# microsoft/tutel

Measured on NVIDIA H100. Metric: moe_layer_fwd_bwd_tokens_per_sec, higher is better.
Workload: dtype bf16; 1 GPU; model=helloworld moe_layer top-2 8-expert ffn(relu) model_dim=4096 hidden=14336, global_batch=16, seq_len=512, parallelism=ep1 (8 local experts/GPU), a2a_ffn_overlap_degree=1, cuda_graph=True, launches_per_graph_replay=15

## Files before the change

### csrc/gemm_sm90.cu

```cuda
#include "gemm_sm90.h"

#include <cuda.h>
#include <cuda_bf16.h>
#include <cuda_fp16.h>

#include <cstdio>
#include <cstdlib>
#include <mutex>

#include "ptx.cuh"

namespace tb {

struct GemmArgs {
  int M, N, K, G;
  int b_group_div;
  int tiles_m, tiles_n;
  long long num_tiles;

  void* d;
  long long ldd, d_group_stride;
  const unsigned long long* d_ptr_table;
  int out_dtype;

// ... 78 lines not shown
  const int first_m = band * kBand;
  const int rows_in_band = min(kBand, tiles_m - first_m);
  r -= band * band_tiles;
  c.m_blk = first_m + r % rows_in_band;
  c.n_blk = r / rows_in_band;
  return c;
}

__device__ __forceinline__ int rotate_group(int g, int rot, int mod) {
  if (mod > 1) {
    const int base = (g / mod) * mod;
    return base + (g - base + rot) % mod;
  }
  if (mod < -1) {
    const int m = -mod;
    const int base = (g / m) * m;
    return base + (rot + m - (g - base)) % m;
  }
  return g;
}

__device__ __forceinline__ float gelu_erf(float x) { return 0.5f * x * (1.0f + erff(x * 0.70710678118654752f)); }
__device__ __forceinline__ float silu(float x) { return __fdividef(x, 1.0f + __expf(-x)); }
__device__ __forceinline__ float fast_sigmoid(float x) { return __fdividef(1.0f, 1.0f + __expf(-x)); }
__device__ __forceinline__ float relu_bwd(float v, float x) { return x > 0.0f ? v : 0.0f; }
__device__ __forceinline__ float gelu_bwd(float v, float x) {
  const float cdf = 0.5f * (1.0f + erff(x * 0.70710678118654752f));
  return v * (cdf + x * 0.3989422804014327f * __expf(-0.5f * x * x));
}
__device__ __forceinline__ float silu_bwd(float v, float x) {
  const float sg = fast_sigmoid(x);
  return v * (sg * (1.0f + x * (1.0f - sg)));
}
__device__ __forceinline__ uint32_t pack2(float a, float b, bool bf16) {
  const __nv_bfloat162 hb = __floats2bfloat162_rn(a, b);
  const __half2 hh = __floats2half2_rn(a, b);
  return bf16 ? *reinterpret_cast<const uint32_t*>(&hb) : *reinterpret_cast<const uint32_t*>(&hh);
}
__device__ __forceinline__ float2 unpack2(uint32_t w, bool bf16) {
  const float2 h = __half22float2(*reinterpret_cast<const __half2*>(&w));
  return bf16 ? make_float2(__uint_as_float(w << 16), __uint_as_float(w & 0xFFFF0000u)) : h;
}

__device__ __forceinline__ void unpack8(const uint4& u, bool is_bf16, float* f) {
  const uint32_t w[4] = {u.x, u.y, u.z, u.w};
#pragma unroll
  for (int i = 0; i < 4; ++i) {
    if (is_bf16) {
      f[2 * i] = __uint_as_float(w[i] << 16);
      f[2 * i + 1] = __uint_as_float(w[i] & 0xFFFF0000u);
    } else {
      const __half2 h = *reinterpret_cast<const __half2*>(&w[i]);
      const float2 t = __half22float2(h);
      f[2 * i] = t.x;
      f[2 * i + 1] = t.y;
    }
  }
}
template <bool BF16>
__device__ __forceinline__ void pack32_t(const float* v, uint32_t* w) {
#pragma unroll
  for (int i = 0; i < 16; ++i) {
    if constexpr (BF16) {
      const __nv_bfloat162 h = __floats2bfloat162_rn(v[2 * i], v[2 * i + 1]);
      w[i] = *reinterpret_cast<const uint32_t*>(&h);
    } else {
      const __half2 h = __floats2half2_rn(v[2 * i], v[2 * i + 1]);
      w[i] = *reinterpret_cast<const uint32_t*>(&h);
    }
  }
}
__device__ __forceinline__ void pack32(const float* v, uint32_t* w, bool is_bf16) {
  if (is_bf16) pack32_t<true>(v, w); else pack32_t<false>(v, w);
}
// ... 29 lines not shown
    else a = g[j] * fast_sigmoid(g[j]);
    o[j] = a * u[j];
  }
}
template <int ACT>
__device__ __forceinline__ void glu_bwd_seg(const float* r, const float* g, float* u, float* o) {
#pragma unroll
  for (int j = 0; j < 32; ++j) {
    const float dh = r[j];
    float a, da;
    if constexpr (ACT == ACT_RELU) {
      a = fmaxf(g[j], 0.0f);
      da = g[j] > 0.0f ? 1.0f : 0.0f;
    } else if constexpr (ACT == ACT_GELU) {
      const float cdf = 0.5f * (1.0f + erff(g[j] * 0.70710678118654752f));
      a = g[j] * cdf;
      da = cdf + g[j] * 0.3989422804014327f * __expf(-0.5f * g[j] * g[j]);
    } else {
      const float sg = fast_sigmoid(g[j]);
      a = g[j] * sg;
      da = sg * (1.0f + g[j] * (1.0f - sg));
    }
    o[j] = dh * u[j] * da;
    u[j] = dh * a;
  }
}

enum WideMain : int { WM_NONE, WM_BIAS, WM_RELU_BWD, WM_ADD, WM_GELU_BWD, WM_SILU_BWD };

__device__ __forceinline__ uint32_t out_tile_off(int j, int swz) {
  return static_cast<uint32_t>((j >> 3) * (128 * kSwizzleBytes) + (((j & 7) ^ swz) << 4));
}

__device__ __forceinline__ void wide_scale(float (&acc)[128], float sa0, float sa1, const float* sb, int n_lane, int n_lim) {
#pragma unroll
  for (int j = 0; j < 32; ++j) {
    const int n = n_lane + 8 * j;
    if (sb != nullptr && n < n_lim) {
      const float2 s = *reinterpret_cast<const float2*>(sb + n);
      acc[4 * j] *= sa0 * s.x; acc[4 * j + 1] *= sa0 * s.y;
      acc[4 * j + 2] *= sa1 * s.x; acc[4 * j + 3] *= sa1 * s.y;
    } else {
      acc[4 * j] *= sa0; acc[4 * j + 1] *= sa0;
      acc[4 * j + 2] *= sa1; acc[4 * j + 3] *= sa1;
    }
  }
}

template <int WM>
__device__ __forceinline__ void wide_main(float (&acc)[128], const uint8_t* row0, int swz, const uint8_t* bias_s,
                                          bool bias_f32, bool bias_bf16, int n_lane, int n_lim, bool out_bf16, float alpha) {
#pragma unroll
  for (int j = 0; j < 32; ++j) {
    if constexpr (WM == WM_NONE) {
#pragma unroll
      for (int c = 0; c < 4; ++c) acc[4 * j + c] *= alpha;
    } else if constexpr (WM == WM_BIAS) {
      const int n = n_lane + 8 * j;
      float2 b = make_float2(0.0f, 0.0f);
      if (n < n_lim)
        b = bias_f32 ? *reinterpret_cast<const float2*>(bias_s + n * 4)
                     : unpack2(*reinterpret_cast<const uint32_t*>(bias_s + n * 2), bias_bf16);
      acc[4 * j] += b.x; acc[4 * j + 1] += b.y;
      acc[4 * j + 2] += b.x; acc[4 * j + 3] += b.y;
    } else {
      const uint32_t o = out_tile_off(j, swz);
#pragma unroll
      for (int h = 0; h < 2; ++h) {
        const float2 f = unpack2(*reinterpret_cast<const uint32_t*>(row0 + h * 8 * kSwizzleBytes + o), out_bf16);
        float& v0 = acc[4 * j + 2 * h];
        float& v1 = acc[4 * j + 2 * h + 1];
        if constexpr (WM == WM_RELU_BWD) { v0 = relu_bwd(v0, f.x); v1 = relu_bwd(v1, f.y); }
        else if constexpr (WM == WM_ADD) { v0 += f.x; v1 += f.y; }
        else if constexpr (WM == WM_GELU_BWD) { v0 = gelu_bwd(v0, f.x); v1 = gelu_bwd(v1, f.y); }
        else { v0 = silu_bwd(v0, f.x); v1 = silu_bwd(v1, f.y); }
      }
    }
  }
}

template <int ACT>
__device__ __forceinline__ void wide_act(float (&acc)[128]) {
#pragma unroll
  for (int i = 0; i < 128; ++i) {
    if constexpr (ACT == ACT_RELU) acc[i] = fmaxf(acc[i], 0.0f);
    else if constexpr (ACT == ACT_GELU) acc[i] = gelu_erf(acc[i]);
    else acc[i] = silu(acc[i]);
  }
}

__device__ __forceinline__ void wide_stage(const float (&acc)[128], uint8_t* row0, int swz, bool out_bf16) {
#pragma unroll
  for (int j = 0; j < 32; ++j) {
    const uint32_t o = out_tile_off(j, swz);
    *reinterpret_cast<uint32_t*>(row0 + o) = pack2(acc[4 * j], acc[4 * j + 1], out_bf16);
    *reinterpret_cast<uint32_t*>(row0 + 8 * kSwizzleBytes + o) = pack2(acc[4 * j + 2], acc[4 * j + 3], out_bf16);
  }
}

template <int OFF>
__device__ __forceinline__ void colsum_halve(float (&s)[64], int lane) {
  const bool upper = (lane & OFF) != 0;
#pragma unroll
  for (int i = 0; i < 2 * OFF; ++i) {
    const float lo = s[i], hi = s[i + 2 * OFF];
    const float recv = __shfl_xor_sync(0xffffffffu, upper ? lo : hi, OFF);
    s[i] = (upper ? hi : lo) + recv;
  }
}
__device__ __forceinline__ void wide_colsum(const float (&acc)[128], bool ok0, bool ok1, int lane, float* colrow) {
  float s[64];
#pragma unroll
  for (int j = 0; j < 32; ++j) {
#pragma unroll
    for (int c = 0; c < 2; ++c) s[2 * j + c] = (ok0 ? acc[4 * j + c] : 0.0f) + (ok1 ? acc[4 * j + 2 + c] : 0.0f);
  }
  colsum_halve<16>(s, lane);
  colsum_halve<8>(s, lane);
  colsum_halve<4>(s, lane);
  float* base = colrow + 32 * (lane >> 2) + 2 * (lane & 3);
#pragma unroll
  for (int q = 0; q < 4; ++q) *reinterpret_cast<float2*>(base + 8 * q) = make_float2(s[2 * q], s[2 * q + 1]);
}

__device__ __forceinline__ void hand_over_tile(const uint8_t* tile, bool straddle, int m0, int n0, int m_valid, int N, int g,
                                               long long group_stride, long long ld, uint8_t* dst, int ct, int lane,
                                               uint32_t out_full) {
  constexpr int kChunks = 256 / 8;
  ptx::fence_proxy_async_smem();
  if (straddle) {
    ptx::named_bar_sync(1, 256);
    for (int i = ct; i < 128 * kChunks; i += 256) {
      const int r = i / kChunks, ch = i % kChunks;
      const int m = m0 + r, n = n0 + ch * 8;
      if (m < m_valid && n < N) {
        const uint4 v = *reinterpret_cast<const uint4*>(tile + (ch >> 3) * (128 * kSwizzleBytes) + r * kSwizzleBytes +
                                                        (((ch & 7) ^ (r & 7)) << 4));
        *reinterpret_cast<uint4*>(dst + (static_cast<long long>(g) * group_stride + static_cast<long long>(m) * ld + n) * 2) = v;
      }
    }
  }
  __syncwarp();
  if (lane == 0) ptx::mbar_arrive(out_full);
}

template <int BN_, bool A_MN, bool B_MN, int DT>
__global__ void __maxnreg__(Cfg<BN_>::MAXNREG)
gemm_sm90_kernel(const __grid_constant__ CUtensorMap tmA, const __grid_constant__ CUtensorMap tmB,
                 const __grid_constant__ CUtensorMap tmB2, const __grid_constant__ CUtensorMap tmD,
                 const __grid_constant__ CUtensorMap tmAux, const __grid_constant__ CUtensorMap tmD2,
                 const GemmArgs args) {
  using C = Cfg<BN_>;
  constexpr int BN = C::BN;
  extern __shared__ uint8_t smem_raw[];

  const int warp = __shfl_sync(0xffffffffu, static_cast<int>(threadIdx.x >> 5), 0);
  const int lane = threadIdx.x & 31;

  const uint32_t smem_base = (ptx::smem_u32(smem_raw) + 1023u) & ~1023u;
  constexpr int stages = C::STAGES;
  const uint32_t out_base = smem_base + static_cast<uint32_t>(stages) * C::STAGE_BYTES;
  const uint32_t bar_base = out_base + C::OUT_TILE_BYTES;
  auto smem_a = [&](int s) { return smem_base + s * C::STAGE_BYTES; };
  auto smem_b = [&](int s) { return smem_base + s * C::STAGE_BYTES + C::A_BYTES; };
  auto full_bar = [&](int s) { return bar_base + 8u * s; };
  auto empty_bar = [&](int s) { return bar_base + 64u + 8u * s; };
  const uint32_t aux_full = bar_base + 128u;
  const uint32_t out_empty = bar_base + 136u;
  const uint32_t out_full = bar_base + 144u;
  auto side_full = [&](uint32_t slot) { return bar_base + 152u + 8u * slot; };
  const uint32_t epi_base = bar_base + C::BAR_BYTES;
  float* epi_ptr = reinterpret_cast<float*>(smem_raw + (epi_base - ptx::smem_u32(smem_raw)));
  uint8_t* out_tile = smem_raw + (out_base - ptx::smem_u32(smem_raw));
  float* colsum_part = epi_ptr;
  const uint32_t side_base = epi_base + C::COLSUM_BYTES;
  const bool aux_tma = C::WIDE && (args.epilogue == EPI_RELU_BWD || args.epilogue == EPI_ADD || args.epilogue == EPI_ACT_BWD);
  const bool side_bias = C::WIDE && args.bias != nullptr && !aux_tma && args.epilogue != EPI_NONE;
  const bool side_in = side_bias || (C::WIDE && args.scale_b != nullptr);
  const bool pre_act = C::WIDE && args.d2 != nullptr && (args.epilogue == EPI_BIAS_GELU || args.epilogue == EPI_BIAS_SILU);
// ... 71 lines not shown
            constexpr int chunk_elems = kSwizzleBytes / kEltBytes;
            constexpr int chunk_bytes = bk_elems * kSwizzleBytes;
            if constexpr (!A_MN) {
              ptx::tma_load_3d(smem_a(s), &tmA, fb, k0, m0, tc.g);
            } else {
              for (int c = 0; c < C::BM / chunk_elems; ++c)
                ptx::tma_load_3d(smem_a(s) + c * chunk_bytes, &tmA, fb, m0 + c * chunk_elems, k0, tc.g);
            }
            if (!dual) {
              if constexpr (!B_MN) {
                ptx::tma_load_3d(smem_b(s), &tmB, fb, k0, n0, gb);
              } else {
                for (int c = 0; c < BN / chunk_elems; ++c)
                  ptx::tma_load_3d(smem_b(s) + c * chunk_bytes, &tmB, fb, n0 + c * chunk_elems, k0, gb);
              }
            } else {
              const int nb0 = tc.n_blk * (BN / 2);
              if constexpr (!B_MN) {
                ptx::tma_load_3d(smem_b(s), &tmB, fb, k0, nb0, gb);
                ptx::tma_load_3d(smem_b(s) + (BN / 2) * kSwizzleBytes, &tmB2, fb, k0, nb0, gb);
              } else {
                constexpr int half_chunks = (BN / 2) / chunk_elems;
                for (int c = 0; c < 2 * half_chunks; ++c)
                  ptx::tma_load_3d(smem_b(s) + c * chunk_bytes, c < half_chunks ? &tmB : &tmB2, fb,
                                   nb0 + (c % half_chunks) * chunk_elems, k0, gb);
              }
            }
          }
          __syncwarp();
          if (++s == stages) { s = 0; ph ^= 1u; }
        }
      }
    } else if (C::WIDE && warp == 1) {
      const int side_es = args.bias_is_fp32 ? 4 : 2;
      uint32_t it = 0;
      uint32_t outs = 0;
      TileCoord prev{};
      int prev_m_valid = 0;
      auto drain = [&](const CUtensorMap* map, const TileCoord& tc, int m_valid, bool colsum, bool has_next, TileCoord next) {
        const int m0 = tc.m_blk * C::BM, n0 = tc.n_blk * BN;
        const bool straddle = m0 + C::BM > m_valid && m_valid < args.M;
        ptx::mbar_wait_quiet(out_full, outs & 1u);
        if (!straddle && lane == 0) {
          for (int b = 0; b < BN / 64; ++b)
            if (n0 + 64 * b < args.N) ptx::tma_store_3d(map, out_base + b * C::OUT_BOX_BYTES, n0 + 64 * b, m0, tc.g);
          ptx::bulk_commit_group();
        }
        if (colsum) {
#pragma unroll 1
          for (int h = 0; h < 2; ++h) {
            const int c = 128 * h + 4 * lane;
            float4 v = *reinterpret_cast<const float4*>(colsum_part + c);
#pragma unroll
            for (int w = 1; w < 8; ++w) {
              const float4 p = *reinterpret_cast<const float4*>(colsum_part + w * BN + c);
              v.x += p.x; v.y += p.y; v.z += p.z; v.w += p.w;
            }
            const int n = n0 + c;
            if (n < args.N) {
              float* cs = args.colsum + static_cast<long long>(tc.g / args.b_group_div) * args.colsum_group_stride + n;
              if ((reinterpret_cast<uintptr_t>(cs) & 15) == 0) {
                ptx::red_add_v4_f32(cs, v.x, v.y, v.z, v.w);
              } else {
                atomicAdd(cs, v.x); atomicAdd(cs + 1, v.y); atomicAdd(cs + 2, v.z); atomicAdd(cs + 3, v.w);
              }
            }
          }
// ... 60 lines not shown
    ptx::setmaxnreg_inc<C::CONSUMER_REGS>();
    const int cw = warp - 4;
    const int wg = cw >> 2;
    const bool wg_leader = (threadIdx.x & 127) == 0;
    int s = 0;
    uint32_t ph = 0;
    constexpr uint32_t kMnChunkBytes = 64u * kSwizzleBytes;
    constexpr uint32_t kMnKStep = 16u * kSwizzleBytes;
    constexpr uint32_t a_lbo = A_MN ? kMnChunkBytes : 16u;
    constexpr uint32_t b_lbo = B_MN ? kMnChunkBytes : 16u;
    constexpr uint32_t a_kstep = (A_MN ? kMnKStep : 32u) >> 4;
    constexpr uint32_t b_kstep = (B_MN ? kMnKStep : 32u) >> 4;
    constexpr uint32_t desc_hi = (1024u >> 4) | (1u << 30);
    const uint32_t a_lo0 = (((smem_a(0) + static_cast<uint32_t>(wg) * 8192u) >> 4) & 0x3FFFu) | ((a_lbo >> 4) << 16);
    const uint32_t b_lo0 = ((smem_b(0) >> 4) & 0x3FFFu) | ((b_lbo >> 4) << 16);

    const bool out16 = (args.out_dtype != DT_FP32);
    const bool out_bf16 = (args.out_dtype == DT_BF16);
    const bool glu = !C::WIDE && (args.epilogue == EPI_GLU || args.epilogue == EPI_GLU_BWD);
    float* epi_warp = epi_ptr + cw * 16 * C::EPI_PITCH;
    const float* epi_row = epi_warp + (lane & 15) * C::EPI_PITCH;
    const int col_half = (lane >> 4) * 32;
    auto load_acc = [&](int col, float* v) {
#pragma unroll
      for (int q = 0; q < 8; ++q) {
        const float4 t4 = *reinterpret_cast<const float4*>(epi_row + col + q * 4);
        v[q * 4] = t4.x; v[q * 4 + 1] = t4.y; v[q * 4 + 2] = t4.z; v[q * 4 + 3] = t4.w;
      }
    };
    const int ct = threadIdx.x - 128;
    const int r0 = cw * 16 + (lane >> 2);
    const int swz = lane >> 2;
    uint8_t* row0 = out_tile + r0 * kSwizzleBytes + (lane & 3) * 4;
    const int wmain = args.epilogue == EPI_NONE ? WM_NONE
                    : args.epilogue == EPI_ADD ? WM_ADD
                    : args.epilogue == EPI_RELU_BWD ? WM_RELU_BWD
                    : args.epilogue == EPI_ACT_BWD ? (args.act == ACT_GELU ? WM_GELU_BWD : args.act == ACT_SILU ? WM_SILU_BWD : WM_RELU_BWD)
                    : WM_BIAS;
    uint32_t it = 0;
    uint32_t outs = 0;

    for (long long t = tile_first; t < args.num_tiles; t += tile_step) {
      TileCoord tc = decode_tile<kBand>(t, args.tiles_m, args.tiles_n);
      tc.g = rotate_group(tc.g, args.group_rot, args.group_mod);
      int m_valid = args.M;
      if (args.row_counts != nullptr) {
        m_valid = min(args.M, args.row_counts[tc.g]);
        if (tc.m_blk * C::BM >= m_valid) continue;
      }
      float acc[BN / 2];
      if constexpr (C::WIDE) {
#pragma unroll
        for (int i = 0; i < BN / 2; ++i) acc[i] = 0.0f;
      }
      int prev_s = 0;
      for (int kb = 0; kb < num_kb; ++kb) {
        ptx::mbar_wait_quiet(full_bar(s), ph);
        const uint32_t a_lo = a_lo0 + static_cast<uint32_t>(s) * (C::STAGE_BYTES >> 4);
        const uint32_t b_lo = b_lo0 + static_cast<uint32_t>(s) * (C::STAGE_BYTES >> 4);
        ptx::wgmma_fence();
#pragma unroll
        for (int k = 0; k < 4; ++k) {
          const uint64_t ad = (static_cast<uint64_t>(desc_hi) << 32) | (a_lo + k * a_kstep);
          const uint64_t bd = (static_cast<uint64_t>(desc_hi) << 32) | (b_lo + k * b_kstep);
          if constexpr (BN == 256) ptx::wgmma_m64n256<DT, A_MN, B_MN>(acc, ad, bd, (kb | k) != 0);
          else ptx::wgmma_m64n128<DT, A_MN, B_MN>(acc, ad, bd, (kb | k) != 0);
        }
        ptx::wgmma_commit();
        if (kb > 0) {
          ptx::wgmma_wait<1>();
          if (wg_leader) ptx::mbar_arrive(empty_bar(prev_s));
        }
        prev_s = s;
        if (++s == stages) { s = 0; ph ^= 1u; }
      }
      ptx::wgmma_wait<0>();
      if (wg_leader) ptx::mbar_arrive(empty_bar(prev_s));

      if constexpr (C::WIDE) {
        const int m0 = tc.m_blk * C::BM, n0 = tc.n_blk * BN;
        const bool ok0 = m0 + r0 < m_valid, ok1 = m0 + r0 + 8 < m_valid;
        const int n_lane = 2 * (lane & 3);
        const int n_lim = args.N - n0;
        const bool straddle = m0 + C::BM > m_valid && m_valid < args.M;
        const uint8_t* side = reinterpret_cast<const uint8_t*>(colsum_part + 8 * BN) + (it & 1u) * C::SIDE_SLOT_BYTES;
        if (side_in) ptx::mbar_wait_quiet(side_full(it & 1u), (it >> 1) & 1u);
        if (args.scale_a != nullptr || args.scale_b != nullptr) {
          const float* sa = args.scale_a != nullptr ? args.scale_a + static_cast<long long>(tc.g) * args.scale_a_group_stride + m0 + r0 : nullptr;
          const float sa0 = (sa != nullptr && ok0) ? sa[0] : 1.0f;
          const float sa1 = (sa != nullptr && ok1) ? sa[8] : 1.0f;
          const float* sb = args.scale_b != nullptr ? reinterpret_cast<const float*>(side + C::SIDE_BIAS_BYTES) : nullptr;
          wide_scale(acc, sa0, sa1, sb, n_lane, n_lim);
        }
        auto wait_out_free = [&]() { ptx::mbar_wait_quiet(out_empty, (outs & 1u) ^ 1u); };
        auto hand_over = [&](uint8_t* dst) {
          hand_over_tile(out_tile, straddle, m0, n0, m_valid, args.N, tc.g, args.d_group_stride, args.ldd, dst, ct, lane, out_full);
          ++outs;
        };

        if (wmain == WM_BIAS) {
          if (side_bias)
            wide_main<WM_BIAS>(acc, row0, swz, side, args.bias_is_fp32 != 0, args.bias_is_bf16 != 0, n_lane, n_lim, out_bf16, 1.0f);
          if (pre_act) {
            wait_out_free();
            wide_stage(acc, row0, swz, out_bf16);
            hand_over(reinterpret_cast<uint8_t*>(args.d2));
          }
          if (args.epilogue == EPI_BIAS_RELU) wide_act<ACT_RELU>(acc);
          else if (args.epilogue == EPI_BIAS_GELU) wide_act<ACT_GELU>(acc);
          else if (args.epilogue == EPI_BIAS_SILU) wide_act<ACT_SILU>(acc);
        } else if (wmain == WM_NONE) {
          if (args.alpha != 1.0f) wide_main<WM_NONE>(acc, row0, swz, nullptr, false, false, n_lane, n_lim, out_bf16, args.alpha);
        } else {
          ptx::mbar_wait_quiet(aux_full, it & 1u);
          if (wmain == WM_RELU_BWD) wide_main<WM_RELU_BWD>(acc, row0, swz, nullptr, false, false, n_lane, n_lim, out_bf16, 1.0f);
          else if (wmain == WM_ADD) wide_main<WM_ADD>(acc, row0, swz, nullptr, false, false, n_lane, n_lim, out_bf16, 1.0f);
          else if (wmain == WM_GELU_BWD) wide_main<WM_GELU_BWD>(acc, row0, swz, nullptr, false, false, n_lane, n_lim, out_bf16, 1.0f);
          else wide_main<WM_SILU_BWD>(acc, row0, swz, nullptr, false, false, n_lane, n_lim, out_bf16, 1.0f);
        }
        if (!aux_tma) wait_out_free();
        wide_stage(acc, row0, swz, out_bf16);
        if (args.colsum != nullptr) wide_colsum(acc, ok0, ok1, lane, colsum_part + cw * BN);
        hand_over(reinterpret_cast<uint8_t*>(args.d));
        ++it;
        continue;
      }

      {
        const int fr = lane >> 2, fc = (lane & 3) * 2;
#pragma unroll
        for (int j = 0; j < C::EPI_COLS / 8; ++j) {
          *reinterpret_cast<float2*>(epi_warp + fr * C::EPI_PITCH + j * 8 + fc) = make_float2(acc[4 * j], acc[4 * j + 1]);
          *reinterpret_cast<float2*>(epi_warp + (fr + 8) * C::EPI_PITCH + j * 8 + fc) = make_float2(acc[4 * j + 2], acc[4 * j + 3]);
        }
      }
      __syncwarp();

      const int m = tc.m_blk * C::BM + cw * 16 + (lane & 15);
      const bool row_ok = m < m_valid;
      const int gb = tc.g / args.b_group_div;
      uint8_t* d_base = (args.d_ptr_table != nullptr)
                            ? reinterpret_cast<uint8_t*>(args.d_ptr_table[tc.g])
                            : reinterpret_cast<uint8_t*>(args.d) +
                                  static_cast<long long>(tc.g) * args.d_group_stride * (out16 ? 2 : 4);
      uint8_t* d_row = d_base + static_cast<long long>(m) * args.ldd * (out16 ? 2 : 4);
      const uint8_t* aux_row = nullptr;
      if (args.aux != nullptr)
        aux_row = reinterpret_cast<const uint8_t*>(args.aux) +
                  (static_cast<long long>(tc.g) * args.aux_group_stride + static_cast<long long>(m) * args.ld_aux) * 2;
      const uint8_t* aux2_row = nullptr;
      if (args.aux2 != nullptr)
        aux2_row = reinterpret_cast<const uint8_t*>(args.aux2) +
                   (static_cast<long long>(tc.g) * args.aux_group_stride + static_cast<long long>(m) * args.ld_aux) * 2;
      const uint8_t* bias_g = nullptr;
      if (args.bias != nullptr)
// ... 234 lines not shown
  }
  dims[2] = static_cast<cuuint64_t>(groups);
  box[2] = 1;
  strides[0] = static_cast<cuuint64_t>(ld) * eb;
  strides[1] = static_cast<cuuint64_t>(groups > 1 ? group_stride : (mn_major ? k : rows_mn) * ld) * eb;
  if (strides[1] == 0) strides[1] = strides[0];
  CUresult r = enc(map, dt, 3, const_cast<void*>(base), dims, strides, box, estr, CU_TENSOR_MAP_INTERLEAVE_NONE,
                   CU_TENSOR_MAP_SWIZZLE_128B, CU_TENSOR_MAP_L2_PROMOTION_L2_256B, CU_TENSOR_MAP_FLOAT_OOB_FILL_NONE);
  if (r != CUDA_SUCCESS) { *why = "cuTensorMapEncodeTiled failed"; return false; }
  return true;
}

bool make_tile_map(CUtensorMap* map, const void* base, int dtype, long long rows, long long cols, long long ld,
                   long long group_stride, int groups, const char** why) {
  EncodeTiledFn enc = get_encode_fn();
  if (enc == nullptr) { *why = "cuTensorMapEncodeTiled unavailable"; return false; }
  if ((reinterpret_cast<uintptr_t>(base) & 15) || ((ld * 2) & 15) || ((group_stride * 2) & 15)) {
    *why = "output / aux base and strides must be 16-byte aligned";
    return false;
  }
  const cuuint64_t dims[3] = {static_cast<cuuint64_t>(cols), static_cast<cuuint64_t>(rows), static_cast<cuuint64_t>(groups)};
  cuuint64_t strides[2] = {static_cast<cuuint64_t>(ld) * 2,
                           static_cast<cuuint64_t>(groups > 1 ? group_stride : rows * ld) * 2};
  if (strides[1] == 0) strides[1] = strides[0];
  const cuuint32_t box[3] = {64, 128, 1};
  const cuuint32_t estr[3] = {1, 1, 1};
  CUresult r = enc(map, dtype == DT_BF16 ? CU_TENSOR_MAP_DATA_TYPE_BFLOAT16 : CU_TENSOR_MAP_DATA_TYPE_FLOAT16, 3,
                   const_cast<void*>(base), dims, strides, box, estr, CU_TENSOR_MAP_INTERLEAVE_NONE,
                   CU_TENSOR_MAP_SWIZZLE_128B, CU_TENSOR_MAP_L2_PROMOTION_L2_256B, CU_TENSOR_MAP_FLOAT_OOB_FILL_NONE);
  if (r != CUDA_SUCCESS) { *why = "cuTensorMapEncodeTiled failed"; return false; }
  return true;
}

template <int BN, bool A_MN, bool B_MN, int DT>
cudaError_t launch_inst(const CUtensorMap& ta, const CUtensorMap& tb_, const CUtensorMap& tb2, const CUtensorMap& td,
                        const CUtensorMap& taux, const CUtensorMap& td2, const GemmArgs& args, int grid,
                        cudaStream_t stream) {
  auto* kern = gemm_sm90_kernel<BN, A_MN, B_MN, DT>;
  static bool configured = false;
  if (!configured) {
    cudaError_t e = cudaFuncSetAttribute(kern, cudaFuncAttributeMaxDynamicSharedMemorySize, Cfg<BN>::SMEM_BYTES);
    if (e != cudaSuccess) return e;
    configured = true;
  }
  kern<<<grid, kThreads, Cfg<BN>::SMEM_BYTES, stream>>>(ta, tb_, tb2, td, taux, td2, args);
  return cudaGetLastError();
}

}

cudaError_t gemm_sm90_launch(const GemmProblem& p, cudaStream_t stream, const char** why_out) {
  const char* why_local = nullptr;
  const char** why = why_out ? why_out : &why_local;
  *why = nullptr;
  if (p.M <= 0 || p.N <= 0 || p.K <= 0 || p.G <= 0) return cudaSuccess;
  const int eb = (p.in_dtype == DT_E4M3 || p.in_dtype == DT_E5M2) ? 1 : 2;
  if (p.N % 8 != 0) { *why = "N must be a multiple of 8"; return cudaErrorInvalidValue; }
  const int ob = p.out_dtype == DT_FP32 ? 4 : 2;
  if ((reinterpret_cast<uintptr_t>(p.d) & 15) || ((p.ldd * ob) & 15) || ((p.d_group_stride * ob) & 15)) {
    *why = "output base/stride must be 16-byte aligned";
    return cudaErrorInvalidValue;
  }

  int dev = 0;
  cudaGetDevice(&dev);
  static int sm_count_cache[64] = {0};
  if (sm_count_cache[dev & 63] == 0) cudaDeviceGetAttribute(&sm_count_cache[dev & 63], cudaDevAttrMultiProcessorCount, dev);
  int sms = sm_count_cache[dev & 63];
  if (p.max_ctas > 0) sms = p.max_ctas < sms ? p.max_ctas : sms;

  const bool dual = p.epilogue == EPI_GLU;
  if (dual && (p.b2 == nullptr || p.out_dtype == DT_FP32)) { *why = "EPI_GLU needs b2 and a 16-bit output"; return cudaErrorInvalidValue; }
  if (p.epilogue == EPI_GLU_BWD && (p.aux == nullptr || p.aux2 == nullptr || p.d2 == nullptr || p.out_dtype == DT_FP32)) {
    *why = "EPI_GLU_BWD needs aux, aux2, d2 and a 16-bit output";
    return cudaErrorInvalidValue;
  }
  if ((p.epilogue == EPI_GLU || p.epilogue == EPI_GLU_BWD) && p.d_ptr_table != nullptr) { *why = "GLU epilogues write local outputs only"; return cudaErrorInvalidValue; }
  const bool uses_aux = p.epilogue == EPI_RELU_BWD || p.epilogue == EPI_ADD || p.epilogue == EPI_GLU_BWD || p.epilogue == EPI_ACT_BWD;
  if (uses_aux && (p.aux == nullptr || p.out_dtype == DT_FP32 ||
                   ((reinterpret_cast<uintptr_t>(p.aux) | reinterpret_cast<uintptr_t>(p.aux2)) & 15) || ((p.ld_aux * 2) & 15) ||
                   ((p.aux_group_stride * 2) & 15))) {
    *why = "this epilogue needs a 16-byte aligned 16-bit aux operand";
    return cudaErrorInvalidValue;
  }
  const int groups_b = (p.G + (p.b_group_div > 0 ? p.b_group_div : 1) - 1) / (p.b_group_div > 0 ? p.b_group_div : 1);
  if ((p.G > 1 && (p.a_group_stride == 0 || (p.d_ptr_table == nullptr && p.d_group_stride == 0) ||
                   (uses_aux && p.aux_group_stride == 0))) ||
      (groups_b > 1 && p.b_group_stride == 0)) {
    *why = "group strides of A, B, aux and the output must be nonzero when there is more than one group";
    return cudaErrorInvalidValue;
  }
  const int mod_abs = p.group_mod < 0 ? -p.group_mod : p.group_mod;
  if (mod_abs > 1 && (p.G % mod_abs != 0 || p.group_rot < 0)) {
    *why = "G must be a multiple of |group_mod|, and group_rot must not be negative";
    return cudaErrorInvalidValue;
  }
  if (p.alpha != 1.0f && p.epilogue != EPI_NONE) { *why = "alpha is applied by EPI_NONE only"; return cudaErrorInvalidValue; }
  if (p.cta_group < 0 || p.cta_group > 2) { *why = "cta_group must be 0, 1 or 2"; return cudaErrorInvalidValue; }
  if (p.block_n != 0 && p.block_n != 128 && p.block_n != 256) { *why = "block_n must be 0, 128 or 256"; return cudaErrorInvalidValue; }

  const bool side_aligned =
      ((reinterpret_cast<uintptr_t>(p.bias) | static_cast<uintptr_t>(p.bias_group_stride * 2)) & 15) == 0 &&
      ((reinterpret_cast<uintptr_t>(p.scale_b) | static_cast<uintptr_t>(p.scale_b_group_stride * 4)) & 15) == 0;
  const bool wide = p.block_n != 128 && p.wait_flags == nullptr && p.signal_ptr_table == nullptr && p.d_ptr_table == nullptr &&
                    p.epilogue != EPI_GLU && p.epilogue != EPI_GLU_BWD && p.out_dtype != DT_FP32 && side_aligned;
  constexpr int bm = 128;
  const int bn = wide ? 256 : 128;
  GemmArgs a{};
  a.M = p.M; a.N = p.N; a.K = p.K; a.G = p.G;
  a.b_group_div = p.b_group_div > 0 ? p.b_group_div : 1;
  a.tiles_m = (p.M + bm - 1) / bm;
  a.tiles_n = dual ? (p.N + bn / 2 - 1) / (bn / 2) : (p.N + bn - 1) / bn;
  a.num_tiles = static_cast<long long>(a.tiles_m) * a.tiles_n * p.G;
  a.d = p.d; a.ldd = p.ldd; a.d_group_stride = p.d_group_stride; a.d_ptr_table = p.d_ptr_table;
  a.out_dtype = p.out_dtype;
  a.epilogue = p.epilogue; a.alpha = p.alpha;
  a.bias = p.bias; a.bias_group_stride = p.bias_group_stride; a.bias_is_fp32 = 0;
  a.bias_is_bf16 = (eb == 2) ? (p.in_dtype == DT_BF16) : (p.out_dtype == DT_BF16);
  a.aux = p.aux; a.ld_aux = p.ld_aux; a.aux_group_stride = p.aux_group_stride;
  a.aux2 = p.aux2; a.d2 = p.d2; a.d3 = p.d3; a.dual = dual ? 1 : 0; a.act = p.act; a.scale_b2 = p.scale_b2;
  a.row_counts = p.row_counts;
  a.colsum = p.colsum; a.colsum_group_stride = p.colsum_group_stride;
  a.scale_a = p.scale_a; a.scale_a_group_stride = p.scale_a_group_stride;
  a.scale_b = p.scale_b; a.scale_b_group_stride = p.scale_b_group_stride;
  a.wait_flags = p.wait_flags; a.wait_rows_per_flag = p.wait_rows_per_flag > 0 ? p.wait_rows_per_flag : bm;
  a.wait_flags_per_group = p.wait_flags_per_group; a.wait_target = p.wait_target;
  a.signal_ptr_table = p.signal_ptr_table;
  a.group_rot = p.group_rot; a.group_mod = p.group_mod;

  CUtensorMap ta, tb_;
  const int gB = (p.G + a.b_group_div - 1) / a.b_group_div;
  if (!make_operand_map(&ta, p.a, p.in_dtype, p.a_mn_major, p.M, p.K, p.lda, p.a_group_stride, p.G, bm, why))
    return cudaErrorInvalidValue;
  const int b_box = dual ? bn / 2 : bn;
  if (!make_operand_map(&tb_, p.b, p.in_dtype, p.b_mn_major, p.N, p.K, p.ldb, p.b_group_stride, gB, b_box, why))
    return cudaErrorInvalidValue;
  CUtensorMap tb2 = tb_;
  if (dual && !make_operand_map(&tb2, p.b2, p.in_dtype, p.b_mn_major, p.N, p.K, p.ldb, p.b_group_stride, gB, b_box, why))
    return cudaErrorInvalidValue;
  CUtensorMap td = tb_, taux = tb_, td2 = tb_;
  if (wide) {
    if (!make_tile_map(&td, p.d, p.out_dtype, p.M, p.N, p.ldd, p.d_group_stride, p.G, why)) return cudaErrorInvalidValue;
    if (uses_aux && !make_tile_map(&taux, p.aux, p.out_dtype, p.M, p.N, p.ld_aux, p.aux_group_stride, p.G, why))
      return cudaErrorInvalidValue;
    if (p.d2 != nullptr && (p.epilogue == EPI_BIAS_GELU || p.epilogue == EPI_BIAS_SILU) &&
        !make_tile_map(&td2, p.d2, p.out_dtype, p.M, p.N, p.ldd, p.d_group_stride, p.G, why))
      return cudaErrorInvalidValue;
  }

  const int grid = static_cast<int>(a.num_tiles < sms ? a.num_tiles : sms);

  if (eb == 1) {
    if (p.a_mn_major || p.b_mn_major) { *why = "fp8 operands must be K-major"; return cudaErrorInvalidValue; }
    const bool xact = p.epilogue == EPI_BIAS_GELU || p.epilogue == EPI_BIAS_SILU || p.epilogue == EPI_ACT_BWD;
    if (xact) { *why = "GELU / SiLU epilogues need 16-bit operands"; return cudaErrorInvalidValue; }
    if (wide) {
      if (p.in_dtype == DT_E4M3) return launch_inst<256, false, false, DT_E4M3>(ta, tb_, tb2, td, taux, td2, a, grid, stream);
      return launch_inst<256, false, false, DT_E5M2>(ta, tb_, tb2, td, taux, td2, a, grid, stream);
    }
    if (p.in_dtype == DT_E4M3) return launch_inst<128, false, false, DT_E4M3>(ta, tb_, tb2, td, taux, td2, a, grid, stream);
    return launch_inst<128, false, false, DT_E5M2>(ta, tb_, tb2, td, taux, td2, a, grid, stream);
  }
#define TB_SWITCH_MAJOR(BNv, DTv)                                                                                  \
  do {                                                                                                             \
    if (!p.a_mn_major && !p.b_mn_major) return launch_inst<BNv, false, false, DTv>(ta, tb_, tb2, td, taux, td2, a, grid, stream);   \
    if (!p.a_mn_major && p.b_mn_major) return launch_inst<BNv, false, true, DTv>(ta, tb_, tb2, td, taux, td2, a, grid, stream);     \
    if (p.a_mn_major && !p.b_mn_major) return launch_inst<BNv, true, false, DTv>(ta, tb_, tb2, td, taux, td2, a, grid, stream);     \
    return launch_inst<BNv, true, true, DTv>(ta, tb_, tb2, td, taux, td2, a, grid, stream);                                        \
  } while (0)
  if (p.in_dtype == DT_BF16) { if (wide) TB_SWITCH_MAJOR(256, DT_BF16); TB_SWITCH_MAJOR(128, DT_BF16); }
  if (p.in_dtype == DT_FP16) { if (wide) TB_SWITCH_MAJOR(256, DT_FP16); TB_SWITCH_MAJOR(128, DT_FP16); }
#undef TB_SWITCH_MAJOR
  *why = "unsupported operand dtype";
  return cudaErrorInvalidValue;
}

cudaError_t set_spin_timeout_gemm(unsigned long long ns) {
  return cudaMemcpyToSymbol(tb_spin_timeout_ns, &ns, sizeof(ns));
}

}
```

### csrc/ptx.cuh

```cuda
#pragma once
#include <cstdint>
#include <cstdio>
#include <cuda.h>
#include <cuda_runtime.h>

#ifndef TB_SPIN_TIMEOUT_NS
#define TB_SPIN_TIMEOUT_NS 300000000000ull
#endif

static __constant__ unsigned long long tb_spin_timeout_ns = TB_SPIN_TIMEOUT_NS;

namespace ptx {

__device__ __forceinline__ uint32_t smem_u32(const void* p) {
  return static_cast<uint32_t>(__cvta_generic_to_shared(p));
}

__device__ __forceinline__ uint64_t globaltimer_ns() {
  uint64_t t;
  asm volatile("mov.u64 %0, %%globaltimer;" : "=l"(t));
  return t;
}

__device__ __forceinline__ uint32_t elect_one() {
// ... 122 lines not shown
    __nanosleep(64);
    if (globaltimer_ns() - t0 > tb_spin_timeout_ns) {
      printf("[tutel_b200] peer flag wait timeout: block %d thread %d flag %p have %u want %u\n", blockIdx.x,
             threadIdx.x, p, ld_relaxed_sys(p), target);
      __trap();
    }
  }
}

__device__ __forceinline__ void wait_flag_ge_sys_quiet(const uint32_t* p, uint32_t target) {
  if (static_cast<int32_t>(ld_acquire_sys(p) - target) >= 0) return;
  const uint64_t t0 = globaltimer_ns();
  while (static_cast<int32_t>(ld_acquire_sys(p) - target) < 0) {
    __nanosleep(64);
    if (globaltimer_ns() - t0 > tb_spin_timeout_ns) __trap();
  }
}

__device__ __forceinline__ uint4 ld_nc_v4(const void* p) {
  uint4 r;
  asm volatile("ld.global.nc.L1::no_allocate.v4.u32 {%0,%1,%2,%3}, [%4];"
               : "=r"(r.x), "=r"(r.y), "=r"(r.z), "=r"(r.w)
               : "l"(p));
  return r;
}
__device__ __forceinline__ uint4 ld_v4(const void* p) {
  uint4 r;
  asm volatile("ld.global.v4.u32 {%0,%1,%2,%3}, [%4];" : "=r"(r.x), "=r"(r.y), "=r"(r.z), "=r"(r.w) : "l"(p));
  return r;
}
__device__ __forceinline__ void st_na_v4(void* p, const uint4& v) {
  asm volatile("st.global.L1::no_allocate.v4.u32 [%0], {%1,%2,%3,%4};" ::"l"(p), "r"(v.x), "r"(v.y), "r"(v.z),
               "r"(v.w)
               : "memory");
}

__device__ __forceinline__ void prefetch_tensormap(const void* tmap) {
  asm volatile("prefetch.tensormap [%0];" ::"l"(tmap) : "memory");
}

__device__ __forceinline__ void tma_load_3d(uint32_t smem_dst, const void* tmap, uint32_t bar, int c0, int c1,
                                            int c2) {
  asm volatile(
      "cp.async.bulk.tensor.3d.shared::cluster.global.mbarrier::complete_tx::bytes"
      " [%0], [%1, {%3, %4, %5}], [%2];" ::"r"(smem_dst),
      "l"(tmap), "r"(bar), "r"(c0), "r"(c1), "r"(c2)
      : "memory");
}
__device__ __forceinline__ void bulk_load(uint32_t smem_dst, const void* gsrc, uint32_t bytes, uint32_t bar) {
  asm volatile("cp.async.bulk.shared::cluster.global.mbarrier::complete_tx::bytes [%0], [%1], %2, [%3];" ::"r"(smem_dst),
               "l"(gsrc), "r"(bytes), "r"(bar)
               : "memory");
}
__device__ __forceinline__ void prefetch_l2_bulk(const void* gptr, uint32_t bytes) {
  asm volatile("cp.async.bulk.prefetch.L2.global [%0], %1;" ::"l"(gptr), "r"(bytes) : "memory");
}

__device__ __forceinline__ void tma_store_3d(const void* tmap, uint32_t smem_src, int c0, int c1, int c2) {
  asm volatile("cp.async.bulk.tensor.3d.global.shared::cta.bulk_group [%0, {%2, %3, %4}], [%1];" ::"l"(tmap),
               "r"(smem_src), "r"(c0), "r"(c1), "r"(c2)
               : "memory");
}
__device__ __forceinline__ void bulk_commit_group() { asm volatile("cp.async.bulk.commit_group;" ::: "memory"); }
template <int N>
__device__ __forceinline__ void bulk_wait_group_read() { asm volatile("cp.async.bulk.wait_group.read %0;" ::"n"(N) : "memory"); }
template <int N>
// ... 86 lines not shown
```

Baseline: 460,100 tokens/s.

## Specialize wide epilogue on output dtype and full tiles, stage via stmatrix

Adds the output dtype as a template parameter of the GEMM kernel, so pack/unpack choose bf16 or fp16 at compile time instead of converting both ways and selecting at runtime. Adds FULL-tile specializations that drop per-column bounds checks in the scale, bias and colsum steps. Replaces the per-element 32-bit shared-memory stores in the wide epilogue staging with stmatrix.x4 instructions. It also restricts the wide path to cases where the output dtype matches the input dtype and drops fp32 bias in that path, which adds template instantiations and code size.

```diff
diff --git a/csrc/gemm_sm90.cu b/csrc/gemm_sm90.cu
--- a/csrc/gemm_sm90.cu
+++ b/csrc/gemm_sm90.cu
@@ -134,14 +134,20 @@
   const float sg = fast_sigmoid(x);
   return v * (sg * (1.0f + x * (1.0f - sg)));
 }
-__device__ __forceinline__ uint32_t pack2(float a, float b, bool bf16) {
-  const __nv_bfloat162 hb = __floats2bfloat162_rn(a, b);
-  const __half2 hh = __floats2half2_rn(a, b);
-  return bf16 ? *reinterpret_cast<const uint32_t*>(&hb) : *reinterpret_cast<const uint32_t*>(&hh);
-}
-__device__ __forceinline__ float2 unpack2(uint32_t w, bool bf16) {
-  const float2 h = __half22float2(*reinterpret_cast<const __half2*>(&w));
-  return bf16 ? make_float2(__uint_as_float(w << 16), __uint_as_float(w & 0xFFFF0000u)) : h;
+template <bool BF16>
+__device__ __forceinline__ uint32_t pack2(float a, float b) {
+  if constexpr (BF16) {
+    const __nv_bfloat162 h = __floats2bfloat162_rn(a, b);
+    return *reinterpret_cast<const uint32_t*>(&h);
+  } else {
+    const __half2 h = __floats2half2_rn(a, b);
+    return *reinterpret_cast<const uint32_t*>(&h);
+  }
+}
+template <bool BF16>
+__device__ __forceinline__ float2 unpack2(uint32_t w) {
+  if constexpr (BF16) return make_float2(__uint_as_float(w << 16), __uint_as_float(w & 0xFFFF0000u));
+  else return __half22float2(*reinterpret_cast<const __half2*>(&w));
 }
 
 __device__ __forceinline__ void unpack8(const uint4& u, bool is_bf16, float* f) {
@@ -237,11 +243,13 @@
   return static_cast<uint32_t>((j >> 3) * (128 * kSwizzleBytes) + (((j & 7) ^ swz) << 4));
 }
 
+
+template <bool FULL>
 __device__ __forceinline__ void wide_scale(float (&acc)[128], float sa0, float sa1, const float* sb, int n_lane, int n_lim) {
 #pragma unroll
   for (int j = 0; j < 32; ++j) {
     const int n = n_lane + 8 * j;
-    if (sb != nullptr && n < n_lim) {
+    if (sb != nullptr && (FULL || n < n_lim)) {
       const float2 s = *reinterpret_cast<const float2*>(sb + n);
       acc[4 * j] *= sa0 * s.x; acc[4 * j + 1] *= sa0 * s.y;
       acc[4 * j + 2] *= sa1 * s.x; acc[4 * j + 3] *= sa1 * s.y;
@@ -252,9 +260,9 @@
   }
 }
 
-template <int WM>
+template <int WM, bool BF16, bool FULL = false>
 __device__ __forceinline__ void wide_main(float (&acc)[128], const uint8_t* row0, int swz, const uint8_t* bias_s,
-                                          bool bias_f32, bool bias_bf16, int n_lane, int n_lim, bool out_bf16, float alpha) {
+                                          int n_lane, int n_lim, float alpha) {
 #pragma unroll
   for (int j = 0; j < 32; ++j) {
     if constexpr (WM == WM_NONE) {
@@ -263,16 +271,14 @@
     } else if constexpr (WM == WM_BIAS) {
       const int n = n_lane + 8 * j;
       float2 b = make_float2(0.0f, 0.0f);
-      if (n < n_lim)
-        b = bias_f32 ? *reinterpret_cast<const float2*>(bias_s + n * 4)
-                     : unpack2(*reinterpret_cast<const uint32_t*>(bias_s + n * 2), bias_bf16);
+      if (FULL || n < n_lim) b = unpack2<BF16>(*reinterpret_cast<const uint32_t*>(bias_s + n * 2));
       acc[4 * j] += b.x; acc[4 * j + 1] += b.y;
       acc[4 * j + 2] += b.x; acc[4 * j + 3] += b.y;
     } else {
       const uint32_t o = out_tile_off(j, swz);
 #pragma unroll
       for (int h = 0; h < 2; ++h) {
-        const float2 f = unpack2(*reinterpret_cast<const uint32_t*>(row0 + h * 8 * kSwizzleBytes + o), out_bf16);
+        const float2 f = unpack2<BF16>(*reinterpret_cast<const uint32_t*>(row0 + h * 8 * kSwizzleBytes + o));
         float& v0 = acc[4 * j + 2 * h];
         float& v1 = acc[4 * j + 2 * h + 1];
         if constexpr (WM == WM_RELU_BWD) { v0 = relu_bwd(v0, f.x); v1 = relu_bwd(v1, f.y); }
@@ -294,12 +300,17 @@
   }
 }
 
-__device__ __forceinline__ void wide_stage(const float (&acc)[128], uint8_t* row0, int swz, bool out_bf16) {
-#pragma unroll
-  for (int j = 0; j < 32; ++j) {
-    const uint32_t o = out_tile_off(j, swz);
-    *reinterpret_cast<uint32_t*>(row0 + o) = pack2(acc[4 * j], acc[4 * j + 1], out_bf16);
-    *reinterpret_cast<uint32_t*>(row0 + 8 * kSwizzleBytes + o) = pack2(acc[4 * j + 2], acc[4 * j + 3], out_bf16);
+template <bool BF16>
+__device__ __forceinline__ void wide_stage(const float (&acc)[128], uint32_t stage_row, int stage_swz, int lane) {
+#pragma unroll
+  for (int p = 0; p < 16; ++p) {
+    uint32_t w[4];
+#pragma unroll
+    for (int q = 0; q < 4; ++q) {
+      const int i = 4 * (2 * p + (q >> 1)) + 2 * (q & 1);
+      w[q] = pack2<BF16>(acc[i], acc[i + 1]);
+    }
+    ptx::stmatrix_x4(stage_row + out_tile_off(2 * p + (lane >> 4), stage_swz), w);
   }
 }
 
@@ -313,12 +324,15 @@
     s[i] = (upper ? hi : lo) + recv;
   }
 }
+template <bool FULL>
 __device__ __forceinline__ void wide_colsum(const float (&acc)[128], bool ok0, bool ok1, int lane, float* colrow) {
   float s[64];
 #pragma unroll
   for (int j = 0; j < 32; ++j) {
 #pragma unroll
-    for (int c = 0; c < 2; ++c) s[2 * j + c] = (ok0 ? acc[4 * j + c] : 0.0f) + (ok1 ? acc[4 * j + 2 + c] : 0.0f);
+    for (int c = 0; c < 2; ++c)
+      s[2 * j + c] = FULL ? acc[4 * j + c] + acc[4 * j + 2 + c]
+                          : (ok0 ? acc[4 * j + c] : 0.0f) + (ok1 ? acc[4 * j + 2 + c] : 0.0f);
   }
   colsum_halve<16>(s, lane);
   colsum_halve<8>(s, lane);
@@ -349,7 +363,7 @@
   if (lane == 0) ptx::mbar_arrive(out_full);
 }
 
-template <int BN_, bool A_MN, bool B_MN, int DT>
+template <int BN_, bool A_MN, bool B_MN, int DT, int OT>
 __global__ void __maxnreg__(Cfg<BN_>::MAXNREG)
 gemm_sm90_kernel(const __grid_constant__ CUtensorMap tmA, const __grid_constant__ CUtensorMap tmB,
                  const __grid_constant__ CUtensorMap tmB2, const __grid_constant__ CUtensorMap tmD,
@@ -487,7 +501,7 @@
         }
       }
     } else if (C::WIDE && warp == 1) {
-      const int side_es = args.bias_is_fp32 ? 4 : 2;
+      constexpr int side_es = 2;
       uint32_t it = 0;
       uint32_t outs = 0;
       TileCoord prev{};
@@ -614,6 +628,9 @@
     const int r0 = cw * 16 + (lane >> 2);
     const int swz = lane >> 2;
     uint8_t* row0 = out_tile + r0 * kSwizzleBytes + (lane & 3) * 4;
+    const int stage_swz = lane & 7;
+    const uint32_t stage_row = out_base + static_cast<uint32_t>(cw * 16 + ((lane >> 3) & 1) * 8 + stage_swz) * kSwizzleBytes;
+    constexpr bool kBf16 = OT == DT_BF16;
     const int wmain = args.epilogue == EPI_NONE ? WM_NONE
                     : args.epilogue == EPI_ADD ? WM_ADD
                     : args.epilogue == EPI_RELU_BWD ? WM_RELU_BWD
@@ -665,6 +682,7 @@
         const int n_lane = 2 * (lane & 3);
         const int n_lim = args.N - n0;
         const bool straddle = m0 + C::BM > m_valid && m_valid < args.M;
+        const bool full = n_lim >= BN && m0 + C::BM <= m_valid;
         const uint8_t* side = reinterpret_cast<const uint8_t*>(colsum_part + 8 * BN) + (it & 1u) * C::SIDE_SLOT_BYTES;
         if (side_in) ptx::mbar_wait_quiet(side_full(it & 1u), (it >> 1) & 1u);
         if (args.scale_a != nullptr || args.scale_b != nullptr) {
@@ -672,7 +690,8 @@
           const float sa0 = (sa != nullptr && ok0) ? sa[0] : 1.0f;
           const float sa1 = (sa != nullptr && ok1) ? sa[8] : 1.0f;
           const float* sb = args.scale_b != nullptr ? reinterpret_cast<const float*>(side + C::SIDE_BIAS_BYTES) : nullptr;
-          wide_scale(acc, sa0, sa1, sb, n_lane, n_lim);
+          if (full) wide_scale<true>(acc, sa0, sa1, sb, n_lane, n_lim);
+          else wide_scale<false>(acc, sa0, sa1, sb, n_lane, n_lim);
         }
         auto wait_out_free = [&]() { ptx::mbar_wait_quiet(out_empty, (outs & 1u) ^ 1u); };
         auto hand_over = [&](uint8_t* dst) {
@@ -681,28 +700,33 @@
         };
 
         if (wmain == WM_BIAS) {
-          if (side_bias)
-            wide_main<WM_BIAS>(acc, row0, swz, side, args.bias_is_fp32 != 0, args.bias_is_bf16 != 0, n_lane, n_lim, out_bf16, 1.0f);
+          if (side_bias) {
+            if (full) wide_main<WM_BIAS, kBf16, true>(acc, row0, swz, side, n_lane, n_lim, 1.0f);
+            else wide_main<WM_BIAS, kBf16, false>(acc, row0, swz, side, n_lane, n_lim, 1.0f);
+          }
           if (pre_act) {
             wait_out_free();
-            wide_stage(acc, row0, swz, out_bf16);
+            wide_stage<kBf16>(acc, stage_row, stage_swz, lane);
             hand_over(reinterpret_cast<uint8_t*>(args.d2));
           }
           if (args.epilogue == EPI_BIAS_RELU) wide_act<ACT_RELU>(acc);
           else if (args.epilogue == EPI_BIAS_GELU) wide_act<ACT_GELU>(acc);
           else if (args.epilogue == EPI_BIAS_SILU) wide_act<ACT_SILU>(acc);
         } else if (wmain == WM_NONE) {
-          if (args.alpha != 1.0f) wide_main<WM_NONE>(acc, row0, swz, nullptr, false, false, n_lane, n_lim, out_bf16, args.alpha);
+          if (args.alpha != 1.0f) wide_main<WM_NONE, kBf16>(acc, row0, swz, nullptr, n_lane, n_lim, args.alpha);
         } else {
           ptx::mbar_wait_quiet(aux_full, it & 1u);
-          if (wmain == WM_RELU_BWD) wide_main<WM_RELU_BWD>(acc, row0, swz, nullptr, false, false, n_lane, n_lim, out_bf16, 1.0f);
-          else if (wmain == WM_ADD) wide_main<WM_ADD>(acc, row0, swz, nullptr, false, false, n_lane, n_lim, out_bf16, 1.0f);
-          else if (wmain == WM_GELU_BWD) wide_main<WM_GELU_BWD>(acc, row0, swz, nullptr, false, false, n_lane, n_lim, out_bf16, 1.0f);
-          else wide_main<WM_SILU_BWD>(acc, row0, swz, nullptr, false, false, n_lane, n_lim, out_bf16, 1.0f);
+          if (wmain == WM_RELU_BWD) wide_main<WM_RELU_BWD, kBf16>(acc, row0, swz, nullptr, n_lane, n_lim, 1.0f);
+          else if (wmain == WM_ADD) wide_main<WM_ADD, kBf16>(acc, row0, swz, nullptr, n_lane, n_lim, 1.0f);
+          else if (wmain == WM_GELU_BWD) wide_main<WM_GELU_BWD, kBf16>(acc, row0, swz, nullptr, n_lane, n_lim, 1.0f);
+          else wide_main<WM_SILU_BWD, kBf16>(acc, row0, swz, nullptr, n_lane, n_lim, 1.0f);
         }
         if (!aux_tma) wait_out_free();
-        wide_stage(acc, row0, swz, out_bf16);
-        if (args.colsum != nullptr) wide_colsum(acc, ok0, ok1, lane, colsum_part + cw * BN);
+        wide_stage<kBf16>(acc, stage_row, stage_swz, lane);
+        if (args.colsum != nullptr) {
+          if (full) wide_colsum<true>(acc, ok0, ok1, lane, colsum_part + cw * BN);
+          else wide_colsum<false>(acc, ok0, ok1, lane, colsum_part + cw * BN);
+        }
         hand_over(reinterpret_cast<uint8_t*>(args.d));
         ++it;
         continue;
@@ -1003,11 +1027,11 @@
   return true;
 }
 
-template <int BN, bool A_MN, bool B_MN, int DT>
+template <int BN, bool A_MN, bool B_MN, int DT, int OT>
 cudaError_t launch_inst(const CUtensorMap& ta, const CUtensorMap& tb_, const CUtensorMap& tb2, const CUtensorMap& td,
                         const CUtensorMap& taux, const CUtensorMap& td2, const GemmArgs& args, int grid,
                         cudaStream_t stream) {
-  auto* kern = gemm_sm90_kernel<BN, A_MN, B_MN, DT>;
+  auto* kern = gemm_sm90_kernel<BN, A_MN, B_MN, DT, OT>;
   static bool configured = false;
   if (!configured) {
     cudaError_t e = cudaFuncSetAttribute(kern, cudaFuncAttributeMaxDynamicSharedMemorySize, Cfg<BN>::SMEM_BYTES);
@@ -1070,11 +1094,12 @@
   if (p.cta_group < 0 || p.cta_group > 2) { *why = "cta_group must be 0, 1 or 2"; return cudaErrorInvalidValue; }
   if (p.block_n != 0 && p.block_n != 128 && p.block_n != 256) { *why = "block_n must be 0, 128 or 256"; return cudaErrorInvalidValue; }
 
+  const bool out_is_in = eb == 1 || p.out_dtype == p.in_dtype;
   const bool side_aligned =
       ((reinterpret_cast<uintptr_t>(p.bias) | static_cast<uintptr_t>(p.bias_group_stride * 2)) & 15) == 0 &&
       ((reinterpret_cast<uintptr_t>(p.scale_b) | static_cast<uintptr_t>(p.scale_b_group_stride * 4)) & 15) == 0;
   const bool wide = p.block_n != 128 && p.wait_flags == nullptr && p.signal_ptr_table == nullptr && p.d_ptr_table == nullptr &&
-                    p.epilogue != EPI_GLU && p.epilogue != EPI_GLU_BWD && p.out_dtype != DT_FP32 && side_aligned;
+                    p.epilogue != EPI_GLU && p.epilogue != EPI_GLU_BWD && p.out_dtype != DT_FP32 && out_is_in && side_aligned;
   constexpr int bm = 128;
   const int bn = wide ? 256 : 128;
   GemmArgs a{};
@@ -1126,18 +1151,23 @@
     const bool xact = p.epilogue == EPI_BIAS_GELU || p.epilogue == EPI_BIAS_SILU || p.epilogue == EPI_ACT_BWD;
     if (xact) { *why = "GELU / SiLU epilogues need 16-bit operands"; return cudaErrorInvalidValue; }
     if (wide) {
-      if (p.in_dtype == DT_E4M3) return launch_inst<256, false, false, DT_E4M3>(ta, tb_, tb2, td, taux, td2, a, grid, stream);
-      return launch_inst<256, false, false, DT_E5M2>(ta, tb_, tb2, td, taux, td2, a, grid, stream);
+      const bool bf16 = p.out_dtype == DT_BF16;
+      if (p.in_dtype == DT_E4M3) {
+        if (bf16) return launch_inst<256, false, false, DT_E4M3, DT_BF16>(ta, tb_, tb2, td, taux, td2, a, grid, stream);
+        return launch_inst<256, false, false, DT_E4M3, DT_FP16>(ta, tb_, tb2, td, taux, td2, a, grid, stream);
+      }
+      if (bf16) return launch_inst<256, false, false, DT_E5M2, DT_BF16>(ta, tb_, tb2, td, taux, td2, a, grid, stream);
+      return launch_inst<256, false, false, DT_E5M2, DT_FP16>(ta, tb_, tb2, td, taux, td2, a, grid, stream);
     }
-    if (p.in_dtype == DT_E4M3) return launch_inst<128, false, false, DT_E4M3>(ta, tb_, tb2, td, taux, td2, a, grid, stream);
-    return launch_inst<128, false, false, DT_E5M2>(ta, tb_, tb2, td, taux, td2, a, grid, stream);
+    if (p.in_dtype == DT_E4M3) return launch_inst<128, false, false, DT_E4M3, DT_BF16>(ta, tb_, tb2, td, taux, td2, a, grid, stream);
+    return launch_inst<128, false, false, DT_E5M2, DT_BF16>(ta, tb_, tb2, td, taux, td2, a, grid, stream);
   }
 #define TB_SWITCH_MAJOR(BNv, DTv)                                                                                  \
   do {                                                                                                             \
-    if (!p.a_mn_major && !p.b_mn_major) return launch_inst<BNv, false, false, DTv>(ta, tb_, tb2, td, taux, td2, a, grid, stream);   \
-    if (!p.a_mn_major && p.b_mn_major) return launch_inst<BNv, false, true, DTv>(ta, tb_, tb2, td, taux, td2, a, grid, stream);     \
-    if (p.a_mn_major && !p.b_mn_major) return launch_inst<BNv, true, false, DTv>(ta, tb_, tb2, td, taux, td2, a, grid, stream);     \
-    return launch_inst<BNv, true, true, DTv>(ta, tb_, tb2, td, taux, td2, a, grid, stream);                                        \
+    if (!p.a_mn_major && !p.b_mn_major) return launch_inst<BNv, false, false, DTv, DTv>(ta, tb_, tb2, td, taux, td2, a, grid, stream); \
+    if (!p.a_mn_major && p.b_mn_major) return launch_inst<BNv, false, true, DTv, DTv>(ta, tb_, tb2, td, taux, td2, a, grid, stream);   \
+    if (p.a_mn_major && !p.b_mn_major) return launch_inst<BNv, true, false, DTv, DTv>(ta, tb_, tb2, td, taux, td2, a, grid, stream);   \
+    return launch_inst<BNv, true, true, DTv, DTv>(ta, tb_, tb2, td, taux, td2, a, grid, stream);                                      \
   } while (0)
   if (p.in_dtype == DT_BF16) { if (wide) TB_SWITCH_MAJOR(256, DT_BF16); TB_SWITCH_MAJOR(128, DT_BF16); }
   if (p.in_dtype == DT_FP16) { if (wide) TB_SWITCH_MAJOR(256, DT_FP16); TB_SWITCH_MAJOR(128, DT_FP16); }
diff --git a/csrc/ptx.cuh b/csrc/ptx.cuh
--- a/csrc/ptx.cuh
+++ b/csrc/ptx.cuh
@@ -178,6 +178,12 @@
 __device__ __forceinline__ void st_na_v4(void* p, const uint4& v) {
   asm volatile("st.global.L1::no_allocate.v4.u32 [%0], {%1,%2,%3,%4};" ::"l"(p), "r"(v.x), "r"(v.y), "r"(v.z),
                "r"(v.w)
+               : "memory");
+}
+
+__device__ __forceinline__ void stmatrix_x4(uint32_t addr, const uint32_t (&r)[4]) {
+  asm volatile("stmatrix.sync.aligned.m8n8.x4.shared.b16 [%0], {%1, %2, %3, %4};" ::"r"(addr), "r"(r[0]), "r"(r[1]),
+               "r"(r[2]), "r"(r[3])
                : "memory");
 }
 
```

Result: faster. 465,800 tokens/s (median of 6 runs) (+1.2%).
